# maybeLx/MVSFormerPlusPlus

Measured on AMD Instinct MI355X. Metric: ref-views/sec at 1152x1536 N=5 D=192 4-stage; achieved HBM GB/s vs peak, higher is better.
Workload: dtype fp16 operands/storage, fp32 accumulate (every stage; 1-2 fp16 MFMA terms)

## Files before the change

### mvsformerplusplus_amd/csrc/conv_bf16x3_kernels.hip

```cpp
#include <map>
#include <mutex>
#include <type_traits>
#include <utility>

#include "conv_cfg.h"
#include "split_format.h"

namespace mvs {

template <class Base>
struct F16Cfg : Base { static constexpr int ACT_F16 = 1; };
template <class Base>
struct F16x1Cfg : Base { static constexpr int ACT_F16 = 2; };
template <class Cfg, class = void> struct CfgFmt { static constexpr bool F16 = false, ONE = false; };
template <class Cfg> struct CfgFmt<Cfg, decltype((void)Cfg::ACT_F16)> { static constexpr bool F16 = true, ONE = Cfg::ACT_F16 == 2; };
typedef _Float16 f16x8 __attribute__((ext_vector_type(8)));
typedef _Float16 f16x4 __attribute__((ext_vector_type(4)));

__device__ __forceinline__ f16x4 f16_pack4(const float4& v, float& amax) {
    const float m = 65504.0f;
    sat::track(amax, v.x, v.y, v.z, v.w);
    return f16x4{(_Float16)__builtin_amdgcn_fmed3f(v.x, -m, m), (_Float16)__builtin_amdgcn_fmed3f(v.y, -m, m),
                 (_Float16)__builtin_amdgcn_fmed3f(v.z, -m, m), (_Float16)__builtin_amdgcn_fmed3f(v.w, -m, m)};
}
// ... 261 lines not shown
            __builtin_amdgcn_sched_barrier(0);
            if constexpr ((T & 1) == 0) bf_mfma_step<Cfg::MREP, Cfg::NREP, CfgFmt<Cfg>::F16, CfgFmt<Cfg>::ONE>(ah, al, bh0, bl0, acc);
            else bf_mfma_step<Cfg::MREP, Cfg::NREP, CfgFmt<Cfg>::F16, CfgFmt<Cfg>::ONE>(ah, al, bh1, bl1, acc);
            if constexpr (T % W::WC == W::WC - 1) {
                if (gc + 1 < nchunk_total) bf_wlds_store<Cfg>(ring, gc + 1, tid, piece);
                __syncthreads();
            }
            BfWldsSteps<Cfg, T + 1>::run(g, lane, tid, wp, ring, gc0, nchunk_total, mb0, ldsb, voxbase0, acc, piece, bh0, bl0, bh1, bl1);
        }
    }
};

template <class Cfg, bool SPLIT>
__global__ __launch_bounds__(256) void conv3d_mfma_bf16x3_kernel(const float* __restrict__ x, const void* wp, const float* __restrict__ bias,
                                                                 float* __restrict__ y, int D, int H, int W, int OD, int OH, int OW,
                                                                 int relu, int tiles_x, int tiles_y, int ntiles) {
    float sat_amax = 0.0f;
    constexpr int CIN = Cfg::CIN, COUT = Cfg::COUT, SD = Cfg::SD, SH = Cfg::SH, SW = Cfg::SW, TD = Cfg::TD, TH = Cfg::TH, CH = Cfg::CH;
    constexpr int IH = Cfg::IH, IW = Cfg::IW, MREP = Cfg::MREP, NREP = Cfg::NREP;
    constexpr int OPT = BfConv<Cfg>::OPT, NSTEP = BfConv<Cfg>::NSTEP, SB = BfConv<Cfg>::SB;
    HIP_DYNAMIC_SHARED(float4, lds4)
    char* ldsb = reinterpret_cast<char*>(lds4);
    const int tid = (int)threadIdx.x, lane = tid & 63, wave = tid >> 6;
    const int li = lane & 15, g = lane >> 4;
    int tile = (int)xcd_remap(blockIdx.x, (unsigned)ntiles);
    const int b = (int)blockIdx.y;
    const int tx = tile % tiles_x;
    tile /= tiles_x;
    const int ty = tile % tiles_y, tz = tile / tiles_y;
    const int oz0 = tz * TD, oy0 = ty * TH, ox0 = tx * 16;
    const int iz0 = oz0 * SD - Cfg::PD, iy0 = oy0 * SH - 1, ix0 = ox0 * SW - 1;

    f32x4 acc[MREP][NREP];
#pragma unroll
    for (int mb = 0; mb < MREP; ++mb)
#pragma unroll
        for (int nb = 0; nb < NREP; ++nb) acc[mb][nb] = (f32x4){0.0f, 0.0f, 0.0f, 0.0f};

    constexpr int MSPLIT = CfgSplit<Cfg>::MSPLIT, MREP_ALL = CfgSplit<Cfg>::MREP_ALL;
    const int mb0 = (wave % MSPLIT) * MREP, rowgrp = wave / MSPLIT;
    int voxbase[NREP];
#pragma unroll
    for (int nb = 0; nb < NREP; ++nb) {
        const int nbg = rowgrp * NREP + nb;
// ... 116 lines not shown
                else bf_conv_load_x<Cfg, T + 1>(g, ldsb, voxbase0, bh0, bl0);
            }
            __builtin_amdgcn_sched_barrier(0);
            const bf16x8* a_hi = BfConv<Cfg>::PERSIST_WLDS ? aw : wh[T];
            const bf16x8* a_lo = BfConv<Cfg>::PERSIST_WLDS ? aw : wl[T];
            if constexpr ((T & 1) == 0) bf_mfma_step<Cfg::MREP, Cfg::NREP, CfgFmt<Cfg>::F16, CfgFmt<Cfg>::ONE>(a_hi, a_lo, bh0, bl0, acc);
            else bf_mfma_step<Cfg::MREP, Cfg::NREP, CfgFmt<Cfg>::F16, CfgFmt<Cfg>::ONE>(a_hi, a_lo, bh1, bl1, acc);
            BfConvStepsWreg<Cfg, T + 1>::run(g, wh, wl, ldsb, voxbase0, acc, bh0, bl0, bh1, bl1, wlane);
        }
    }
};

template <class Cfg, bool SPLIT>
__global__ __launch_bounds__(256) void conv3d_mfma_bf16x3_persist_kernel(const float* __restrict__ x, const void* wp, const float* __restrict__ bias,
                                                                         float* __restrict__ y, float* __restrict__ logits, int D, int H, int W,
                                                                         int OD, int OH, int OW, int relu, int tiles_x, int tiles_y, int ntiles) {
    float sat_amax = 0.0f;
    constexpr int CIN = Cfg::CIN, COUT = Cfg::COUT, SD = Cfg::SD, SH = Cfg::SH, SW = Cfg::SW, TD = Cfg::TD, TH = Cfg::TH;
    constexpr int IH = Cfg::IH, IW = Cfg::IW, MREP = Cfg::MREP, NREP = Cfg::NREP;
    constexpr int OPT = BfConv<Cfg>::OPT, NSTEP = BfConv<Cfg>::NSTEP, SB = BfConv<Cfg>::SB;
    static_assert(Cfg::NPASS == 1, "the persistent form keeps one channel chunk's weights in registers");
    HIP_DYNAMIC_SHARED(float4, lds4)
    char* ldsb = reinterpret_cast<char*>(lds4);
    const int tid = (int)threadIdx.x, lane = tid & 63, wave = tid >> 6;
    const int li = lane & 15, g = lane >> 4;
    const int b = (int)blockIdx.y;
    const int nblk = (int)gridDim.x, per = (ntiles + nblk - 1) / nblk;
    const int t_begin = (int)xcd_remap(blockIdx.x, (unsigned)nblk) * per;
    const int t_end = t_begin + per < ntiles ? t_begin + per : ntiles;
    if (t_begin >= t_end) return;

    const bf16x8* wq = reinterpret_cast<const bf16x8*>(wp) + lane;
    bf16x8 wh[NSTEP][MREP], wl[NSTEP][MREP];
    constexpr bool WL = BfConv<Cfg>::PERSIST_WLDS;
    const char* wlane = ldsb + BfConv<Cfg>::WLDS_OFF + lane * 16;
    if constexpr (WL) {
        bf16x8* dst = reinterpret_cast<bf16x8*>(ldsb + BfConv<Cfg>::WLDS_OFF);
        for (int i = tid; i < NSTEP * MREP * 64; i += 256) dst[i] = reinterpret_cast<const bf16x8*>(wp)[(size_t)((i >> 6) * 2) * 64 + (i & 63)];
    } else {
#pragma unroll
        for (int t = 0; t < NSTEP; ++t)
#pragma unroll
            for (int mb = 0; mb < MREP; ++mb) {
                wh[t][mb] = wq[(size_t)((t * MREP + mb) * 2) * 64];
// ... 7 lines not shown
    int voxbase[NREP];
#pragma unroll
    for (int nb = 0; nb < NREP; ++nb) {
        const int nbg = wave * NREP + nb;
        const int oz = nbg / TH, oy = nbg % TH;
        voxbase[nb] = (((oz * SD) * IH + oy * SH) * IW + li * SW) * SB;
    }
    constexpr bool F16 = BfConv<Cfg>::F16;
    constexpr int EB = F16 ? 2 : 4, RUNB = BfConv<Cfg>::RUNB;
    const char* xb = reinterpret_cast<const char*>(x) + (size_t)b * D * H * W * CIN * EB;
    char* yb = y ? reinterpret_cast<char*>(y) + (size_t)b * OD * OH * OW * COUT * EB : nullptr;

    constexpr int NITEM = Cfg::NVOX * OPT, NIT = (NITEM + 255) / 256;
    float4 su[NIT], sv[NIT];
    auto issue = [&](int tile) {
        const int tx = tile % tiles_x;
        const int t1 = tile / tiles_x;
        const int ty = t1 % tiles_y, tz = t1 / tiles_y;
        const int iz0 = tz * TD * SD - Cfg::PD, iy0 = ty * TH * SH - 1, ix0 = tx * 16 * SW - 1;
        int zrel;
        const __amdgpu_buffer_rsrc_t xrs = bf_make_rsrc_z(xb, iz0, D, H, W, (unsigned)(CIN * EB), zrel);
        BfTileWalk<IW, IH, OPT, RUNB> wk(tid, zrel, iy0, ix0, H, W, CIN * EB, 0u);
#pragma unroll
        for (int it = 0; it < NIT; ++it) {
            if (it > 0) wk.advance();
            const bool ok = (it * 256 + 255 < NITEM || tid + it * 256 < NITEM) && wk.inside(iz0, iy0, ix0, D, H, W);
            const unsigned voff = ok ? wk.off : BF_OOB;
            su[it] = bf_buf_load16(xrs, voff, 0);
            if constexpr (!F16) sv[it] = bf_buf_load16(xrs, voff, 16);
        }
    };
    auto process = [&](int tile) {
#pragma unroll
        for (int it = 0; it < NIT; ++it) {
            const int e = tid + it * 256;
            if (e >= NITEM) break;
            const int vox = e / OPT, oc = e - vox * OPT;
            if constexpr (F16) *reinterpret_cast<float4*>(ldsb + vox * SB + oc * BfConv<Cfg>::PLANE) = su[it];
            else stage_to_lds<SPLIT>(ldsb + vox * SB + oc * BfConv<Cfg>::PLANE, su[it], sv[it]);
        }
        __syncthreads();
        if (tile + 1 < t_end) issue(tile + 1);

        f32x4 acc[MREP][NREP];
#pragma unroll
        for (int mb = 0; mb < MREP; ++mb)
#pragma unroll
            for (int nb = 0; nb < NREP; ++nb) acc[mb][nb] = (f32x4){0.0f, 0.0f, 0.0f, 0.0f};
        {
            bf16x8 bh0[NREP], bl0[NREP], bh1[NREP], bl1[NREP];
            bf_conv_load_x<Cfg, 0>(g, ldsb, voxbase[0], bh0, bl0);
            BfConvStepsWreg<Cfg, 0>::run(g, wh, wl, ldsb, voxbase[0], acc, bh0, bl0, bh1, bl1, wlane);
        }

        const int tx = tile % tiles_x;
        const int t1 = tile / tiles_x;
        const int ty = t1 % tiles_y, tz = t1 / tiles_y;
        const int oz0 = tz * TD, oy0 = ty * TH, ox0 = tx * 16;
#pragma unroll
        for (int nb = 0; nb < NREP; ++nb) {
            const int nbg = wave * NREP + nb;
            const int oz = oz0 + nbg / TH, oy = oy0 + nbg % TH, ox = ox0 + li;
            const bool inside = oz < OD && oy < OH && ox < OW;
            if (!inside && (!SPLIT || logits != nullptr)) continue;
            if (logits != nullptr) {
                if (g == 0) logits[(size_t)b * OD * OH * OW + ((size_t)oz * OH + oy) * OW + ox] = acc[0][nb][0] + bb[0].x;
                continue;
            }
            float* o = reinterpret_cast<float*>(yb + (((size_t)oz * OH + oy) * OW + ox) * COUT * EB);
#pragma unroll
            for (int mb = 0; mb < MREP; ++mb) {
                const int co = 16 * mb + 4 * g;
                if (!SPLIT && co >= COUT) continue;
                float4 v = make_float4(acc[mb][nb][0] + bb[mb].x, acc[mb][nb][1] + bb[mb].y, acc[mb][nb][2] + bb[mb].z, acc[mb][nb][3] + bb[mb].w);
                if (relu) { v.x = fmaxf(v.x, 0.0f); v.y = fmaxf(v.y, 0.0f); v.z = fmaxf(v.z, 0.0f); v.w = fmaxf(v.w, 0.0f); }
                if constexpr (F16) *reinterpret_cast<f16x4*>(reinterpret_cast<_Float16*>(o) + co) = f16_pack4(v, sat_amax);
                else if (SPLIT) split_store_quad(o + (co & ~7), g, v, inside && co < COUT);
                else *reinterpret_cast<float4*>(o + co) = v;
            }
        }
        __syncthreads();
    };
    issue(t_begin);
    for (int tile = t_begin; tile < t_end; ++tile) process(tile);
    if constexpr (F16) sat::commit(sat_amax);
}


template <class Cfg>
struct BfDeconv {
    static constexpr int OPT = Cfg::CIN / 8;
    static constexpr bool F16 = CfgFmt<Cfg>::F16;
    static constexpr int RUNB = F16 ? 16 : 32;
    static constexpr int SB = F16 ? 16 : 32;
    static constexpr int PLANE = F16 ? (Cfg::NVOX * 16 + 255) / 256 * 256 + bf_f16_plane_shift(1)
                                     : (Cfg::NVOX * 32 + 255) / 256 * 256 + 16;
    static constexpr size_t LDS_BYTES = (size_t)OPT * PLANE;
};

// ... 125 lines not shown
            bfdf_mfma_all<Cfg, U, P::F16 ? 1 : 2>(ah, al, bh[U & 1], bl[U & 1], acc);
            if constexpr (NEXT) {
                __builtin_amdgcn_sched_barrier(0);
                bfdf_load_w_all<Cfg, U + 1, 2, 1>(wrs, wvoff, ah, al);
            }
            BfDeconvFSteps<Cfg, U + 1>::run(wrs, wvoff, px, acc, ah, al, bh, bl);
        }
    }
};

template <class Cfg, bool SPLIT, bool FUSED = false>
__global__ __launch_bounds__(256) void deconv3d_mfma_bf16x3_kernel(const float* __restrict__ x, const void* wp, const float* __restrict__ bias,
                                                                   const float* __restrict__ skip, float* __restrict__ y,
                                                                   const float* __restrict__ prob_w, const float* __restrict__ prob_b,
                                                                   float* __restrict__ logits, int D, int H, int W, int tiles_x,
                                                                   int tiles_y, int ntiles, int relu) {
    float sat_amax = 0.0f;
    constexpr int CIN = Cfg::CIN, COUT = Cfg::COUT, SD = Cfg::SD, TDM = Cfg::TDM, THM = Cfg::THM;
    constexpr int LH = Cfg::LH, LW = Cfg::LW, MREP = Cfg::MREP, NREP = Cfg::NREP;
    constexpr int OPT = BfDeconv<Cfg>::OPT, SB = BfDeconv<Cfg>::SB;
    const float lo_clamp = relu ? 0.0f : -INFINITY;
    HIP_DYNAMIC_SHARED(float4, lds4)
    char* ldsb = reinterpret_cast<char*>(lds4);
    const int tid = (int)threadIdx.x, lane = tid & 63, wave = tid >> 6;
    const int li = lane & 15, g = lane >> 4;
    int tile = (int)xcd_remap(blockIdx.x, (unsigned)ntiles);
    const int b = (int)blockIdx.y;
    const int tx = tile % tiles_x;
    tile /= tiles_x;
    const int ty = tile % tiles_y, tz = tile / tiles_y;
    const int mz0 = tz * TDM, my0 = ty * THM, mx0 = tx * 16;
    const int OD = D * SD, OH = 2 * H, OW = 2 * W;

    constexpr bool F16 = BfDeconv<Cfg>::F16;
    constexpr int EB = F16 ? 2 : 4, RUNB = BfDeconv<Cfg>::RUNB;
    const char* xb = reinterpret_cast<const char*>(x) + (size_t)b * D * H * W * CIN * EB;
    {
        int zrel;
        const __amdgpu_buffer_rsrc_t xrs = bf_make_rsrc_z(xb, mz0 - Cfg::ZO, D, H, W, (unsigned)(CIN * EB), zrel);
        BfTileWalk<LW, LH, OPT, RUNB> wk(tid, zrel, my0, mx0, H, W, CIN * EB, 0u);
        int ldso = (tid / OPT) * SB + (tid % OPT) * BfDeconv<Cfg>::PLANE;
        for (int e = tid; e < Cfg::NVOX * OPT; e += 256) {
            const bool ok = wk.inside(mz0 - Cfg::ZO, my0, mx0, D, H, W);
            const unsigned voff = ok ? wk.off : BF_OOB;
            const float4 u = bf_buf_load16(xrs, voff, 0);
// ... 222 lines not shown
                else bfd_load_step<Cfg, IT, T + 1>(g, lane, ldsx, ldsw, voxbase0, a0[0], a0[1], bh0, bl0);
            }
            __builtin_amdgcn_sched_barrier(0);
            if constexpr ((T & 1) == 0) bf_mfma_step<1, Cfg::NREP, CfgFmt<Cfg>::F16, CfgFmt<Cfg>::ONE>(&a0[0], &a0[1], bh0, bl0, acc);
            else bf_mfma_step<1, Cfg::NREP, CfgFmt<Cfg>::F16, CfgFmt<Cfg>::ONE>(&a1[0], &a1[1], bh1, bl1, acc);
            BfDeconvSteps<Cfg, IT, T + 1>::run(g, lane, ldsx, ldsw, voxbase0, acc, a0, bh0, bl0, a1, bh1, bl1);
        }
    }
};

template <class Cfg, bool SPLIT>
__global__ __launch_bounds__(256) void deconv3d_mfma_bf16x3_persist_kernel(const float* __restrict__ x, const void* wp, const float* __restrict__ bias,
                                                                           const float* __restrict__ skip, float* __restrict__ y,
                                                                           const float* __restrict__ prob_w, const float* __restrict__ prob_b,
                                                                           float* __restrict__ logits, int D, int H, int W, int tiles_x, int tiles_y,
                                                                           int ntiles, int relu) {
    float sat_amax = 0.0f;
    using P = BfDeconvP<Cfg>;
    const float lo_clamp = relu ? 0.0f : -INFINITY;
    constexpr int CIN = Cfg::CIN, COUT = Cfg::COUT, SD = Cfg::SD, TDM = Cfg::TDM, THM = Cfg::THM;
    constexpr int LH = Cfg::LH, LW = Cfg::LW, NREP = Cfg::NREP, NIT = P::NIT, OPT = P::OPT, SB = P::SB;
    HIP_DYNAMIC_SHARED(float4, lds4)
    char* ldsx = reinterpret_cast<char*>(lds4);
    char* ldsw = ldsx + P::XBYTES;
    const int tid = (int)threadIdx.x, lane = tid & 63, wave = tid >> 6;
    const int li = lane & 15, g = lane >> 4;
    const int b = (int)blockIdx.y;
    const int nblk = (int)gridDim.x, per = (ntiles + nblk - 1) / nblk;
    const int t_begin = (int)xcd_remap(blockIdx.x, (unsigned)nblk) * per;
    const int t_end = t_begin + per < ntiles ? t_begin + per : ntiles;
    if (t_begin >= t_end) return;
    const int OD = D * SD, OH = 2 * H, OW = 2 * W;

    for (int e = tid; e < P::WBYTES / 16; e += 256) reinterpret_cast<float4*>(ldsw)[e] = reinterpret_cast<const float4*>(wp)[e];

    constexpr bool F16 = P::F16;
    constexpr int EB = F16 ? 2 : 4;
    const char* xb = reinterpret_cast<const char*>(x) + (size_t)b * D * H * W * CIN * EB;
    float* yb = y ? reinterpret_cast<float*>(reinterpret_cast<char*>(y) + (size_t)b * OD * OH * OW * COUT * EB) : nullptr;
    const float* sb = skip ? reinterpret_cast<const float*>(reinterpret_cast<const char*>(skip) + (size_t)b * OD * OH * OW * COUT * EB) : nullptr;
    const int co = 4 * (g & 1);
    const float4 bb = *reinterpret_cast<const float4*>(bias + co);
    const bool head = prob_w != nullptr;
    const float4 pw4 = head ? *reinterpret_cast<const float4*>(prob_w + co) : make_float4(0.0f, 0.0f, 0.0f, 0.0f);
    const float pb = head ? prob_b[0] : 0.0f;

    int voxbase[NREP];
#pragma unroll
    for (int nb = 0; nb < NREP; ++nb) {
        const int nbg = wave * NREP + nb;
        const int mz = nbg / THM, my = nbg % THM;
        voxbase[nb] = (((mz + Cfg::ZO) * LH + my) * LW + li) * SB;
    }

    constexpr int NITEM = Cfg::NVOX * OPT, NITX = (NITEM + 255) / 256;
    float4 su[NITX], sv[NITX];
    auto issue_x = [&](int tile) {
        const int tx = tile % tiles_x;
        const int t1 = tile / tiles_x;
        const int ty = t1 % tiles_y, tz = t1 / tiles_y;
        const int mz0 = tz * TDM, my0 = ty * THM, mx0 = tx * 16;
        int zrel;
        const __amdgpu_buffer_rsrc_t xrs = bf_make_rsrc_z(xb, mz0 - Cfg::ZO, D, H, W, (unsigned)(CIN * EB), zrel);
        BfTileWalk<LW, LH, OPT, P::RUNB> wk(tid, zrel, my0, mx0, H, W, CIN * EB, 0u);
#pragma unroll
        for (int it = 0; it < NITX; ++it) {
            if (it > 0) wk.advance();
            const bool ok = (it * 256 + 255 < NITEM || tid + it * 256 < NITEM) && wk.inside(mz0 - Cfg::ZO, my0, mx0, D, H, W);
            const unsigned voff = ok ? wk.off : BF_OOB;
            su[it] = bf_buf_load16(xrs, voff, 0);
            if constexpr (!F16) sv[it] = bf_buf_load16(xrs, voff, 16);
        }
    };
    float4 skp[NIT][NREP];
    auto issue_skip = [&](int tile) {
        const int tx = tile % tiles_x;
        const int t1 = tile / tiles_x;
        const int ty = t1 % tiles_y, tz = t1 / tiles_y;
        const int mz0 = tz * TDM, my0 = ty * THM, mx0 = tx * 16;
#pragma unroll
        for (int it = 0; it < NIT; ++it) {
            const int pd = (SD == 2) ? (it >> 1) : 0, ph = it & 1;
#pragma unroll
            for (int nb = 0; nb < NREP; ++nb) {
                const int nbg = wave * NREP + nb;
                const int mz = mz0 + nbg / THM, my = my0 + nbg % THM, mx = mx0 + li;
                const bool inside = mz < D && my < H && mx < W;
                const int oz = mz * SD + pd, oy = 2 * my + ph, ox = 2 * mx + (g >> 1);
                const size_t vbase = inside ? (((size_t)oz * OH + oy) * OW + ox) * COUT : 0;
                if constexpr (F16) {
                    const float2 raw = *reinterpret_cast<const float2*>(reinterpret_cast<const _Float16*>(sb) + vbase + co);
                    skp[it][nb] = inside ? make_float4(raw.x, raw.y, 0.0f, 0.0f) : make_float4(0.0f, 0.0f, 0.0f, 0.0f);
                    continue;
                }
                const float4 sk = SPLIT ? split_raw_quad(sb + vbase, co >> 2) : *reinterpret_cast<const float4*>(sb + vbase + co);
                skp[it][nb] = inside ? sk : make_float4(0.0f, 0.0f, 0.0f, 0.0f);
            }
        }
    };
    issue_x(t_begin);
    if (sb) issue_skip(t_begin);
    for (int tile = t_begin; tile < t_end; ++tile) {
#pragma unroll
        for (int it = 0; it < NITX; ++it) {
            const int e = tid + it * 256;
            if (e >= NITEM) break;
            const int vox = e / OPT, oc = e - vox * OPT;
            if constexpr (F16) *reinterpret_cast<float4*>(ldsx + vox * SB + oc * P::PLANE) = su[it];
            else stage_to_lds<SPLIT>(ldsx + vox * SB + oc * P::PLANE, su[it], sv[it]);
        }
        __syncthreads();
        if (tile + 1 < t_end) issue_x(tile + 1);

        const int tx = tile % tiles_x;
        const int t1 = tile / tiles_x;
        const int ty = t1 % tiles_y, tz = t1 / tiles_y;
        const int mz0 = tz * TDM, my0 = ty * THM, mx0 = tx * 16;
        float4 outv[NIT][NREP];
        auto run_class = [&](auto itc) {
            constexpr int IT = decltype(itc)::value;
            f32x4 acc[1][NREP];
#pragma unroll
            for (int nb = 0; nb < NREP; ++nb) acc[0][nb] = (f32x4){0.0f, 0.0f, 0.0f, 0.0f};
            bf16x8 a0[2], a1[2], bh0[NREP], bl0[NREP], bh1[NREP], bl1[NREP];
            bfd_load_step<Cfg, IT, 0>(g, lane, ldsx, ldsw, voxbase[0], a0[0], a0[1], bh0, bl0);
            BfDeconvSteps<Cfg, IT, 0>::run(g, lane, ldsx, ldsw, voxbase[0], acc, a0, bh0, bl0, a1, bh1, bl1);
#pragma unroll
            for (int nb = 0; nb < NREP; ++nb)
                outv[IT][nb] = make_float4(fmaxf(acc[0][nb][0] + bb.x, lo_clamp), fmaxf(acc[0][nb][1] + bb.y, lo_clamp), fmaxf(acc[0][nb][2] + bb.z, lo_clamp),
                                           fmaxf(acc[0][nb][3] + bb.w, lo_clamp));
        };
// ... 23 lines not shown
                    part += v.z * pw4.z;
                    part += v.w * pw4.w;
                    part += __shfl_xor(part, 16);
                    if ((g & 1) == 0 && inside)
                        logits[(size_t)b * OD * OH * OW + ((size_t)oz * OH + oy) * OW + ox] = part + pb;
                } else if (F16) {
                    if (inside) *reinterpret_cast<f16x4*>(reinterpret_cast<_Float16*>(yb) + (((size_t)oz * OH + oy) * OW + ox) * COUT + co) =
                        f16_pack4(v, sat_amax);
                } else if (SPLIT) {
                    split_store_quad(yb + (((size_t)oz * OH + oy) * OW + ox) * COUT, g, v, inside);
                } else if (inside) {
                    *reinterpret_cast<float4*>(yb + (((size_t)oz * OH + oy) * OW + ox) * COUT + co) = v;
                }
            }
        }
        if (sb && tile + 1 < t_end) issue_skip(tile + 1);
        __syncthreads();
    }
    if constexpr (F16) sat::commit(sat_amax);
}

static int resident_blocks(const void* func, size_t lds, int threads = 256) {
    static std::mutex mu;
    static std::map<std::pair<const void*, int>, int> cache;
    int dev = 0;
    if (hipGetDevice(&dev) != hipSuccess) return -1;
    std::lock_guard<std::mutex> lock(mu);
    auto it = cache.find(std::make_pair(func, dev));
    if (it != cache.end()) return it->second;
    int per_cu = 0;
    hipDeviceProp_t prop;
    if (lds > 48 * 1024) hipFuncSetAttribute(func, hipFuncAttributeMaxDynamicSharedMemorySize, (int)lds);
    if (hipGetDeviceProperties(&prop, dev) != hipSuccess || hipOccupancyMaxActiveBlocksPerMultiprocessor(&per_cu, func, threads, lds) != hipSuccess || per_cu < 1)
        return -1;
    return cache[std::make_pair(func, dev)] = per_cu * prop.multiProcessorCount;
}

constexpr int BF_MSPLIT_MIN_MREP = 4;
template <class Cfg>
struct BfSplitOf {
    static constexpr bool SPLIT = Cfg::MREP >= BF_MSPLIT_MIN_MREP && Cfg::NREP <= 2 && Cfg::TH % (Cfg::NREP * 2) == 0;
    typedef typename std::conditional<SPLIT, SplitCfg<Cfg, 2>, Cfg>::type type;
};

template <class Cfg, bool SPLIT>
static int launch_conv_bf(const float* x, const void* wp, const float* bias, float* y, int B, int D, int H, int W, int relu, hipStream_t st,
                          float* logits) {
    const int OD = (D + 2 * Cfg::PD - Cfg::KD) / Cfg::SD + 1, OH = (H - 1) / Cfg::SH + 1, OW = (W - 1) / Cfg::SW + 1;
    const int tx = (int)ceil_div(OW, 16), ty = (int)ceil_div(OH, Cfg::TH), tz = (int)ceil_div(OD, Cfg::TD);
    const int ntiles = tx * ty * tz;
    constexpr size_t LDS = BfConv<Cfg>::PERSIST ? BfConv<Cfg>::PERSIST_LDS_BYTES : BfConv<Cfg>::LDS_BYTES;
    if constexpr (BfConv<Cfg>::PERSIST) {
        const int resident = resident_blocks(reinterpret_cast<const void*>(&conv3d_mfma_bf16x3_persist_kernel<Cfg, SPLIT>), LDS);
        if (resident < 1) { set_error("conv3d(bf16x3): occupancy query failed"); return MVS_ERR_LAUNCH; }
        const int nblk = ntiles < resident ? ntiles : resident;
        hipLaunchKernelGGL((conv3d_mfma_bf16x3_persist_kernel<Cfg, SPLIT>), dim3(nblk, B), dim3(256), LDS, st, x, wp, bias, y, logits, D, H, W, OD, OH, OW, relu, tx,
                           ty, ntiles);
        return check_launch("conv3d_mfma_bf16x3_persist_kernel");
    }
    if (logits != nullptr) { set_error("conv3d(bf16x3): the planar single-channel output needs a persistent (Cin = 8) kernel"); return MVS_ERR_UNSUPPORTED; }
    constexpr size_t TLDS = BfWlds<Cfg>::ENABLED ? BfWlds<Cfg>::LDS_BYTES : LDS;
    if (TLDS > 48 * 1024)
        hipFuncSetAttribute(reinterpret_cast<const void*>(&conv3d_mfma_bf16x3_kernel<Cfg, SPLIT>), hipFuncAttributeMaxDynamicSharedMemorySize, (int)TLDS);
    hipLaunchKernelGGL((conv3d_mfma_bf16x3_kernel<Cfg, SPLIT>), dim3(ntiles, B), dim3(256), TLDS, st, x, wp, bias, y, D, H, W, OD, OH, OW, relu, tx, ty, ntiles);
    return check_launch("conv3d_mfma_bf16x3_kernel");
}

template <class Cfg>
struct BfDeconvSplitOf {
    static constexpr bool SPLIT = Cfg::MREP == 2 && Cfg::THM % (Cfg::NREP * 2) == 0;
    typedef typename std::conditional<SPLIT, SplitCfg<Cfg, 2>, Cfg>::type type;
};

template <class Cfg, bool SPLIT>
static int launch_deconv_bf(const float* x, const void* wp, const float* bias, const float* skip, float* y, const float* prob_w,
                            const float* prob_b, float* logits, int B, int D, int H, int W, hipStream_t st, int relu) {
    const int tx = (int)ceil_div(W, 16), ty = (int)ceil_div(H, Cfg::THM), tz = (int)ceil_div(D, Cfg::TDM);
    const int ntiles = tx * ty * tz;
    if constexpr (Cfg::CIN == 16 && Cfg::COUT == 8) {
        constexpr size_t LDS = BfDeconvP<Cfg>::LDS_BYTES;
        const int resident = resident_blocks(reinterpret_cast<const void*>(&deconv3d_mfma_bf16x3_persist_kernel<Cfg, SPLIT>), LDS);
        if (resident < 1) { set_error("deconv3d(bf16x3): occupancy query failed"); return MVS_ERR_LAUNCH; }
        const int nblk = ntiles < resident ? ntiles : resident;
        hipLaunchKernelGGL((deconv3d_mfma_bf16x3_persist_kernel<Cfg, SPLIT>), dim3(nblk, B), dim3(256), LDS, st, x, wp, bias, skip, y, prob_w, prob_b, logits, D, H,
                           W, tx, ty, ntiles, relu);
        return check_launch("deconv3d_mfma_bf16x3_persist_kernel");
    }
    constexpr size_t DLDS = BfDeconv<Cfg>::LDS_BYTES;
    if constexpr (BfDeconvF<Cfg>::ENABLED) {
        const char* sw = getenv("MVS_DECONV_CLASS_FUSED");
        const bool fused = (sw == nullptr || sw[0] == '\0') ? BfDeconvF<Cfg>::DEFAULT : sw[0] != '0';
        if (fused) {
            if (DLDS > 48 * 1024)
                hipFuncSetAttribute(reinterpret_cast<const void*>(&deconv3d_mfma_bf16x3_kernel<Cfg, SPLIT, true>), hipFuncAttributeMaxDynamicSharedMemorySize, (int)DLDS);
            hipLaunchKernelGGL((deconv3d_mfma_bf16x3_kernel<Cfg, SPLIT, true>), dim3(ntiles, B), dim3(256), DLDS, st, x, wp, bias, skip, y, prob_w, prob_b,
                               logits, D, H, W, tx, ty, ntiles, relu);
            return check_launch("deconv3d_mfma_bf16x3_kernel");
        }
    }
    if (DLDS > 48 * 1024)
        hipFuncSetAttribute(reinterpret_cast<const void*>(&deconv3d_mfma_bf16x3_kernel<Cfg, SPLIT>), hipFuncAttributeMaxDynamicSharedMemorySize, (int)DLDS);
    hipLaunchKernelGGL((deconv3d_mfma_bf16x3_kernel<Cfg, SPLIT>), dim3(ntiles, B), dim3(256), DLDS, st, x, wp, bias, skip, y, prob_w, prob_b,
                       logits, D, H, W, tx, ty, ntiles, relu);
    return check_launch("deconv3d_mfma_bf16x3_kernel");
}

static bool bf_input_fits(const char* who, int Cin, int D, int H, int W, int split) {
    const long long bytes = 12LL * H * W * Cin * (split >= 2 ? 2 : 4);
    if (bytes < (1LL << 31)) return true;
    set_error("%s: twelve z-planes of the input are %lld bytes; the MFMA convolutions address a tile's planes with 32-bit offsets (< 2 GB)", who, bytes);
    return false;
}

int conv3d_dispatch_bf16x3(const float* x, const void* wp, const float* bias, float* y, int B, int Cin, int Cout, int D, int H, int W,
                           int kd, int sd, int sh, int sw, int relu, hipStream_t st, float* logits, int split) {
    if (!bf_input_fits("conv3d(mfma)", Cin, D, H, W, split)) return MVS_ERR_UNSUPPORTED;
#define MVS_X(CI, CO, KD, SD, SH, SW, TD, TH, CH)                                                     \
    if (Cin == CI && Cout == CO && kd == KD && sd == SD && sh == SH && sw == SW) {                    \
// ... 34 lines not shown
```

### mvsformerplusplus_amd/csrc/head_kernels.hip

```cpp
#include "mvs_common.h"

namespace mvs {

template <int DC>
__device__ __forceinline__ void head_from_logits(const float* l, const float* lg, const float* hp, size_t HW, int D, float tmp, int mode, int conf_n,
                                                 float* pv, float& depth, float& conf) {
#define HL(d) (DC > 0 ? l[(DC > 0 ? (d) : 0)] : lg[(size_t)(d) * HW])
    float m = -INFINITY;
#pragma unroll
    for (int d = 0; d < D; ++d) m = fmaxf(m, HL(d));
    float den = 0.0f;
#pragma unroll
    for (int d = 0; d < D; ++d) den += expf(HL(d) - m);

    depth = 0.0f;
    conf = 0.0f;
    if (mode == MVS_HEAD_CE_EVAL) {
        float m2 = -INFINITY;
#pragma unroll
        for (int d = 0; d < D; ++d) m2 = fmaxf(m2, HL(d) * tmp);
        float den2 = 0.0f;
#pragma unroll
        for (int d = 0; d < D; ++d) den2 += expf(HL(d) * tmp - m2);
#pragma unroll
// ... 224 lines not shown
            const float dmax = dep + (float)D / 2.0f * itv;
            lo[k] = dmin;
            span[k] = (dmax - dmin) / (float)(D - 1);
        }
    }
    for (int d = 0; d < D; ++d) {
        float c[4];
#pragma unroll
        for (int k = 0; k < 4; ++k)
            c[k] = linear ? lo[k] + (float)d * span[k] : lo[k] + span[k] * ((float)d / (float)(D - 1));
        const float v = ly0 * (lx0 * c[0] + lx1 * c[1]) + ly1 * (lx0 * c[2] + lx1 * c[3]);
        hyp[((size_t)b * D + d) * HW + p] = linear ? v : 1.0f / v;
    }
}

constexpr int HS_SH = 8, HS_SW = 32, HS_RH = HS_SH + 2, HS_RW = HS_SW + 2, HS_NREG = HS_RH * HS_RW;

template <int DC>
__global__ __launch_bounds__(256) void prob_regress_sched_kernel(const float* __restrict__ logits, const float* __restrict__ hyp, float tmp, int mode,
                                                                 int conf_n, float* __restrict__ depth_out, float* __restrict__ conf_out,
                                                                 float* __restrict__ prob_vol, int D_, int H, int W, float ratio,
                                                                 float* __restrict__ next_hyp, int Dn, int tiles_x) {
    __shared__ float s_lo[HS_NREG], s_span[HS_NREG];
    const int D = DC > 0 ? DC : D_;
    const size_t HW = (size_t)H * W;
    const int b = (int)blockIdx.y;
    const int ty = (int)blockIdx.x / tiles_x, tx = (int)blockIdx.x - ty * tiles_x;
    const int y0 = ty * HS_SH, x0 = tx * HS_SW;
    for (int task = (int)threadIdx.x; task < HS_NREG; task += 256) {
        const int ry = task / HS_RW, rx = task - ry * HS_RW;
        const int y = y0 - 1 + ry, x = x0 - 1 + rx;
        if (y < 0 || y >= H || x < 0 || x >= W) continue;
        const bool owner = ry >= 1 && ry <= HS_SH && rx >= 1 && rx <= HS_SW;
        const size_t p = (size_t)y * W + x;
        const float* lg = logits + (size_t)b * D * HW + p;
        const float* hp = hyp + (size_t)b * D * HW + p;
        float l[DC > 0 ? DC : 1];
        if (DC > 0) {
#pragma unroll
            for (int d = 0; d < (DC > 0 ? DC : 1); ++d) l[d] = lg[(size_t)d * HW];
        }
        float depth, conf;
// ... 134 lines not shown
        if (!cp.p[i] || cp.shift[i] < 0 || cp.shift[i] > 16 || ((H >> cp.shift[i]) << cp.shift[i]) != H || ((W >> cp.shift[i]) << cp.shift[i]) != W) {
            set_error("mvs_softmax_regress_confavg_fwd: earlier stage %d must be a 2^shift-times smaller map of this %dx%d stage", i, H, W);
            return MVS_ERR_ARG;
        }
    return launch_head<0>(logits, nullptr, nullptr, hyp, tmp, mode, conf_n, depth, conf, prob_volume, const_cast<float*>(logits), B, D, H, W, (hipStream_t)stream, cp, conf_avg);
}

extern "C" int mvs_softmax_regress_schedule_fwd(const float* logits, const float* hyp, float tmp, int mode, int conf_n, float* depth, float* conf,
                                               float* prob_volume, float ratio, float* next_hyp, int next_D, int B, int D, int H, int W, void* stream) {
    int rc = check_head("mvs_softmax_regress_schedule_fwd", logits, hyp, depth, conf, mode, B, D, H, W);
    if (rc != MVS_OK) return rc;
    if (!next_hyp || next_D < 2 || D < 3 || H < 2 || W < 2) { set_error("mvs_softmax_regress_schedule_fwd: bad arguments (needs D >= 3 hypotheses, module.py:708, and next_D >= 2)"); return MVS_ERR_ARG; }
    const int tiles_x = (int)ceil_div(W, HS_SW), tiles_y = (int)ceil_div(H, HS_SH);
    const dim3 grid(tiles_x * tiles_y, B), block(256);
    hipStream_t st = (hipStream_t)stream;
#define MVS_HS_CASE(DC)                                                                                                                   \
    case DC:                                                                                                                              \
        hipLaunchKernelGGL((prob_regress_sched_kernel<DC>), grid, block, 0, st, logits, hyp, tmp, mode, conf_n, depth, conf, prob_volume, D, H, W, ratio, \
                           next_hyp, next_D, tiles_x);                                                                                    \
        break;
    switch (D) {
        MVS_HS_CASE(4)
        MVS_HS_CASE(8)
        MVS_HS_CASE(16)
        MVS_HS_CASE(32)
        MVS_HS_CASE(48)
        default:
            hipLaunchKernelGGL((prob_regress_sched_kernel<0>), grid, block, 0, st, logits, hyp, tmp, mode, conf_n, depth, conf, prob_volume, D, H, W, ratio,
                               next_hyp, next_D, tiles_x);
    }
#undef MVS_HS_CASE
    return check_launch("prob_regress_sched_kernel");
}

extern "C" int mvs_depth_regression_fwd(const float* p, const float* depth_values, float* out, int B, int D, int H, int W, void* stream) {
    if (!p || !depth_values || !out || B < 1 || D < 1 || H < 1 || W < 1) { set_error("mvs_depth_regression_fwd: bad arguments"); return MVS_ERR_ARG; }
    hipLaunchKernelGGL(depth_regression_kernel, dim3(ceil_div((long long)H * W, 256), B), dim3(256), 0, (hipStream_t)stream, p, depth_values, out, D, H * W);
    return check_launch("depth_regression_kernel");
}

extern "C" int mvs_conf_regression_fwd(const float* p, int n, float* out, int B, int D, int H, int W, void* stream) {
    if (!p || !out || n < 1 || B < 1 || D < 1 || H < 1 || W < 1) { set_error("mvs_conf_regression_fwd: bad arguments"); return MVS_ERR_ARG; }
    hipLaunchKernelGGL(conf_regression_kernel, dim3(ceil_div((long long)H * W, 256), B), dim3(256), 0, (hipStream_t)stream, p, n, out, D, H * W);
    return check_launch("conf_regression_kernel");
// ... 58 lines not shown
```

### mvsformerplusplus_amd/csrc/mvs_common.h

```cpp
#pragma once
#include <hip/hip_runtime.h>

#include <stdint.h>

#include "../../include/mvs_hip.h"

#ifndef MVS_GLOBAL_LOAD_LDS16
#define MVS_GLOBAL_LOAD_LDS16(gsrc, ldst) \
    __builtin_amdgcn_global_load_lds((const __attribute__((address_space(1))) void*)(gsrc), (__attribute__((address_space(3))) void*)(ldst), 16, 0, 0)
#define MVS_WAIT_VMEM() asm volatile("s_waitcnt vmcnt(0)" ::: "memory")
#endif

#ifndef MVS_FMA_MIX_LO
namespace mvs {
__device__ __forceinline__ float fma_mix_lo(unsigned h2, float w, float acc) {
    float r;
    asm("v_fma_mix_f32 %0, %1, %2, %3 op_sel_hi:[1,0,0]" : "=v"(r) : "v"(h2), "v"(w), "v"(acc));
    return r;
}
__device__ __forceinline__ float fma_mix_hi(unsigned h2, float w, float acc) {
    float r;
    asm("v_fma_mix_f32 %0, %1, %2, %3 op_sel:[1,0,0] op_sel_hi:[1,0,0]" : "=v"(r) : "v"(h2), "v"(w), "v"(acc));
    return r;
}
// ... 28 lines not shown
}
#define MVS_DEFINE_SAT_READER(fn)                                                        \
    unsigned int fn(int reset) {                                                         \
        unsigned int v = 0;                                                              \
        if (hipMemcpyFromSymbol(&v, HIP_SYMBOL(mvs::sat::counter), sizeof(v)) != hipSuccess) return 0; \
        if (reset && v) { const unsigned int z = 0; hipMemcpyToSymbol(HIP_SYMBOL(mvs::sat::counter), &z, sizeof(z)); } \
        return v;                                                                        \
    }

constexpr int kWave = 64;
constexpr int kBlock = 256;
constexpr int kMaxSrcViews = 16;

void set_error(const char* fmt, ...);
int check_launch(const char* what);

template <int DT> struct FeatT;
template <> struct FeatT<MVS_DTYPE_F32> { typedef float type; };
template <> struct FeatT<MVS_DTYPE_BF16> { typedef uint16_t type; };
template <> struct FeatT<MVS_DTYPE_F16> { typedef _Float16 type; };

__device__ __forceinline__ float to_f32(float v) { return v; }
__device__ __forceinline__ float to_f32(_Float16 v) { return (float)v; }
__device__ __forceinline__ float to_f32(uint16_t bf16_bits) {
    union { uint32_t u; float f; } c;
    c.u = ((uint32_t)bf16_bits) << 16;
    return c.f;
}

template <typename T> __device__ __forceinline__ T from_f32(float v);
// ... 132 lines not shown
    int xb = x0, yb = y0;
    float wa = wx0, wb = wx1, wt = wy0, wd = wy1;
    if ((unsigned)x0 > (unsigned)(W - 2) || (unsigned)y0 > (unsigned)(H - 2)) {
        xb = x0 < 0 ? 0 : (x0 > W - 2 ? W - 2 : x0);
        yb = y0 < 0 ? 0 : (y0 > H - 2 ? H - 2 : y0);
        wa = x0 < 0 ? wx1 : (x0 > W - 2 ? 0.0f : wx0);
        wb = x0 < 0 ? 0.0f : (x0 > W - 2 ? wx0 : wx1);
        wt = y0 < 0 ? wy1 : (y0 > H - 2 ? 0.0f : wy0);
        wd = y0 < 0 ? 0.0f : (y0 > H - 2 ? wy0 : wy1);
    }
    tp.pk = ((unsigned)yb << 16) | (unsigned)xb;
    tp.w00 = wa * wt; tp.w01 = wb * wt; tp.w10 = wa * wd; tp.w11 = wb * wd;
    return tp;
}

__device__ __forceinline__ unsigned xcd_remap(unsigned b, unsigned n) {
    const unsigned q = n >> 3, r = n & 7u, xcd = b & 7u, idx = b >> 3;
    const unsigned base = (xcd < r) ? xcd * (q + 1) : r * (q + 1) + (xcd - r) * q;
    return base + idx;
}

static inline unsigned ceil_div(long long a, long long b) { return (unsigned)((a + b - 1) / b); }

__device__ __forceinline__ float init_range_value(float first, float last, int inverse, int d, int D) {
    if (inverse) {
        const float inv_min = 1.0f / first, inv_max = 1.0f / last;
        const float itv = (float)d / (float)(D - 1);
        return 1.0f / (inv_max + (inv_min - inv_max) * itv);
    }
    const float interval = (last - first) / (float)(D - 1);
    return first + (float)d * interval;
}

}
```

Baseline: 700.8.

## Reorder conv/deconv/head tiles into row bands for cross-XCD cache locality

Adds a banded tile ordering: tiles are decoded so that a few rows of y, spanning all x and z tiles, are handled together. The band height is sized so each band's working set fits in about 1 MiB of cache. Persistent kernels now take tiles with a stride inside an XCD group instead of a contiguous run. The goal is more L2/MALL reuse of halo rows between neighbouring tiles on the same XCD, which should cut HBM traffic. It is on by default for selected configs, can be switched off with an environment variable, and adds index arithmetic per tile plus a different load balance.

```diff
diff --git a/mvsformerplusplus_amd/csrc/conv_bf16x3_kernels.hip b/mvsformerplusplus_amd/csrc/conv_bf16x3_kernels.hip
--- a/mvsformerplusplus_amd/csrc/conv_bf16x3_kernels.hip
+++ b/mvsformerplusplus_amd/csrc/conv_bf16x3_kernels.hip
@@ -299,7 +299,7 @@
 template <class Cfg, bool SPLIT>
 __global__ __launch_bounds__(256) void conv3d_mfma_bf16x3_kernel(const float* __restrict__ x, const void* wp, const float* __restrict__ bias,
                                                                  float* __restrict__ y, int D, int H, int W, int OD, int OH, int OW,
-                                                                 int relu, int tiles_x, int tiles_y, int ntiles) {
+                                                                 int relu, int tiles_x, int tiles_y, int tiles_z, int band) {
     float sat_amax = 0.0f;
     constexpr int CIN = Cfg::CIN, COUT = Cfg::COUT, SD = Cfg::SD, SH = Cfg::SH, SW = Cfg::SW, TD = Cfg::TD, TH = Cfg::TH, CH = Cfg::CH;
     constexpr int IH = Cfg::IH, IW = Cfg::IW, MREP = Cfg::MREP, NREP = Cfg::NREP;
@@ -308,11 +308,9 @@
     char* ldsb = reinterpret_cast<char*>(lds4);
     const int tid = (int)threadIdx.x, lane = tid & 63, wave = tid >> 6;
     const int li = lane & 15, g = lane >> 4;
-    int tile = (int)xcd_remap(blockIdx.x, (unsigned)ntiles);
     const int b = (int)blockIdx.y;
-    const int tx = tile % tiles_x;
-    tile /= tiles_x;
-    const int ty = tile % tiles_y, tz = tile / tiles_y;
+    int tx, ty, tz;
+    tile_decode((int)xcd_remap(blockIdx.x, gridDim.x), tiles_x, tiles_y, tiles_z, band, tx, ty, tz);
     const int oz0 = tz * TD, oy0 = ty * TH, ox0 = tx * 16;
     const int iz0 = oz0 * SD - Cfg::PD, iy0 = oy0 * SH - 1, ix0 = ox0 * SW - 1;
 
@@ -459,7 +457,8 @@
 template <class Cfg, bool SPLIT>
 __global__ __launch_bounds__(256) void conv3d_mfma_bf16x3_persist_kernel(const float* __restrict__ x, const void* wp, const float* __restrict__ bias,
                                                                          float* __restrict__ y, float* __restrict__ logits, int D, int H, int W,
-                                                                         int OD, int OH, int OW, int relu, int tiles_x, int tiles_y, int ntiles) {
+                                                                         int OD, int OH, int OW, int relu, int tiles_x, int tiles_y, int tiles_z,
+                                                                         int band) {
     float sat_amax = 0.0f;
     constexpr int CIN = Cfg::CIN, COUT = Cfg::COUT, SD = Cfg::SD, SH = Cfg::SH, SW = Cfg::SW, TD = Cfg::TD, TH = Cfg::TH;
     constexpr int IH = Cfg::IH, IW = Cfg::IW, MREP = Cfg::MREP, NREP = Cfg::NREP;
@@ -470,9 +469,8 @@
     const int tid = (int)threadIdx.x, lane = tid & 63, wave = tid >> 6;
     const int li = lane & 15, g = lane >> 4;
     const int b = (int)blockIdx.y;
-    const int nblk = (int)gridDim.x, per = (ntiles + nblk - 1) / nblk;
-    const int t_begin = (int)xcd_remap(blockIdx.x, (unsigned)nblk) * per;
-    const int t_end = t_begin + per < ntiles ? t_begin + per : ntiles;
+    const TileRun trun = tile_run((int)blockIdx.x, (int)gridDim.x, tiles_x * tiles_y * tiles_z, band);
+    const int t_begin = trun.first, t_end = trun.end, t_step = trun.stride;
     if (t_begin >= t_end) return;
 
     const bf16x8* wq = reinterpret_cast<const bf16x8*>(wp) + lane;
@@ -510,9 +508,8 @@
     constexpr int NITEM = Cfg::NVOX * OPT, NIT = (NITEM + 255) / 256;
     float4 su[NIT], sv[NIT];
     auto issue = [&](int tile) {
-        const int tx = tile % tiles_x;
-        const int t1 = tile / tiles_x;
-        const int ty = t1 % tiles_y, tz = t1 / tiles_y;
+        int tx, ty, tz;
+        tile_decode(tile, tiles_x, tiles_y, tiles_z, band, tx, ty, tz);
         const int iz0 = tz * TD * SD - Cfg::PD, iy0 = ty * TH * SH - 1, ix0 = tx * 16 * SW - 1;
         int zrel;
         const __amdgpu_buffer_rsrc_t xrs = bf_make_rsrc_z(xb, iz0, D, H, W, (unsigned)(CIN * EB), zrel);
@@ -536,7 +533,7 @@
             else stage_to_lds<SPLIT>(ldsb + vox * SB + oc * BfConv<Cfg>::PLANE, su[it], sv[it]);
         }
         __syncthreads();
-        if (tile + 1 < t_end) issue(tile + 1);
+        if (tile + t_step < t_end) issue(tile + t_step);
 
         f32x4 acc[MREP][NREP];
 #pragma unroll
@@ -549,9 +546,8 @@
             BfConvStepsWreg<Cfg, 0>::run(g, wh, wl, ldsb, voxbase[0], acc, bh0, bl0, bh1, bl1, wlane);
         }
 
-        const int tx = tile % tiles_x;
-        const int t1 = tile / tiles_x;
-        const int ty = t1 % tiles_y, tz = t1 / tiles_y;
+        int tx, ty, tz;
+        tile_decode(tile, tiles_x, tiles_y, tiles_z, band, tx, ty, tz);
         const int oz0 = tz * TD, oy0 = ty * TH, ox0 = tx * 16;
 #pragma unroll
         for (int nb = 0; nb < NREP; ++nb) {
@@ -578,7 +574,7 @@
         __syncthreads();
     };
     issue(t_begin);
-    for (int tile = t_begin; tile < t_end; ++tile) process(tile);
+    for (int tile = t_begin; tile < t_end; tile += t_step) process(tile);
     if constexpr (F16) sat::commit(sat_amax);
 }
 
@@ -734,7 +730,7 @@
                                                                    const float* __restrict__ skip, float* __restrict__ y,
                                                                    const float* __restrict__ prob_w, const float* __restrict__ prob_b,
                                                                    float* __restrict__ logits, int D, int H, int W, int tiles_x,
-                                                                   int tiles_y, int ntiles, int relu) {
+                                                                   int tiles_y, int tiles_z, int band, int relu) {
     float sat_amax = 0.0f;
     constexpr int CIN = Cfg::CIN, COUT = Cfg::COUT, SD = Cfg::SD, TDM = Cfg::TDM, THM = Cfg::THM;
     constexpr int LH = Cfg::LH, LW = Cfg::LW, MREP = Cfg::MREP, NREP = Cfg::NREP;
@@ -744,11 +740,9 @@
     char* ldsb = reinterpret_cast<char*>(lds4);
     const int tid = (int)threadIdx.x, lane = tid & 63, wave = tid >> 6;
     const int li = lane & 15, g = lane >> 4;
-    int tile = (int)xcd_remap(blockIdx.x, (unsigned)ntiles);
     const int b = (int)blockIdx.y;
-    const int tx = tile % tiles_x;
-    tile /= tiles_x;
-    const int ty = tile % tiles_y, tz = tile / tiles_y;
+    int tx, ty, tz;
+    tile_decode((int)xcd_remap(blockIdx.x, gridDim.x), tiles_x, tiles_y, tiles_z, band, tx, ty, tz);
     const int mz0 = tz * TDM, my0 = ty * THM, mx0 = tx * 16;
     const int OD = D * SD, OH = 2 * H, OW = 2 * W;
 
@@ -1001,7 +995,7 @@
                                                                            const float* __restrict__ skip, float* __restrict__ y,
                                                                            const float* __restrict__ prob_w, const float* __restrict__ prob_b,
                                                                            float* __restrict__ logits, int D, int H, int W, int tiles_x, int tiles_y,
-                                                                           int ntiles, int relu) {
+                                                                           int tiles_z, int band, int relu) {
     float sat_amax = 0.0f;
     using P = BfDeconvP<Cfg>;
     const float lo_clamp = relu ? 0.0f : -INFINITY;
@@ -1013,9 +1007,8 @@
     const int tid = (int)threadIdx.x, lane = tid & 63, wave = tid >> 6;
     const int li = lane & 15, g = lane >> 4;
     const int b = (int)blockIdx.y;
-    const int nblk = (int)gridDim.x, per = (ntiles + nblk - 1) / nblk;
-    const int t_begin = (int)xcd_remap(blockIdx.x, (unsigned)nblk) * per;
-    const int t_end = t_begin + per < ntiles ? t_begin + per : ntiles;
+    const TileRun trun = tile_run((int)blockIdx.x, (int)gridDim.x, tiles_x * tiles_y * tiles_z, band);
+    const int t_begin = trun.first, t_end = trun.end, t_step = trun.stride;
     if (t_begin >= t_end) return;
     const int OD = D * SD, OH = 2 * H, OW = 2 * W;
 
@@ -1043,9 +1036,8 @@
     constexpr int NITEM = Cfg::NVOX * OPT, NITX = (NITEM + 255) / 256;
     float4 su[NITX], sv[NITX];
     auto issue_x = [&](int tile) {
-        const int tx = tile % tiles_x;
-        const int t1 = tile / tiles_x;
-        const int ty = t1 % tiles_y, tz = t1 / tiles_y;
+        int tx, ty, tz;
+        tile_decode(tile, tiles_x, tiles_y, tiles_z, band, tx, ty, tz);
         const int mz0 = tz * TDM, my0 = ty * THM, mx0 = tx * 16;
         int zrel;
         const __amdgpu_buffer_rsrc_t xrs = bf_make_rsrc_z(xb, mz0 - Cfg::ZO, D, H, W, (unsigned)(CIN * EB), zrel);
@@ -1061,9 +1053,8 @@
     };
     float4 skp[NIT][NREP];
     auto issue_skip = [&](int tile) {
-        const int tx = tile % tiles_x;
-        const int t1 = tile / tiles_x;
-        const int ty = t1 % tiles_y, tz = t1 / tiles_y;
+        int tx, ty, tz;
+        tile_decode(tile, tiles_x, tiles_y, tiles_z, band, tx, ty, tz);
         const int mz0 = tz * TDM, my0 = ty * THM, mx0 = tx * 16;
 #pragma unroll
         for (int it = 0; it < NIT; ++it) {
@@ -1087,7 +1078,7 @@
     };
     issue_x(t_begin);
     if (sb) issue_skip(t_begin);
-    for (int tile = t_begin; tile < t_end; ++tile) {
+    for (int tile = t_begin; tile < t_end; tile += t_step) {
 #pragma unroll
         for (int it = 0; it < NITX; ++it) {
             const int e = tid + it * 256;
@@ -1097,11 +1088,10 @@
             else stage_to_lds<SPLIT>(ldsx + vox * SB + oc * P::PLANE, su[it], sv[it]);
         }
         __syncthreads();
-        if (tile + 1 < t_end) issue_x(tile + 1);
-
-        const int tx = tile % tiles_x;
-        const int t1 = tile / tiles_x;
-        const int ty = t1 % tiles_y, tz = t1 / tiles_y;
+        if (tile + t_step < t_end) issue_x(tile + t_step);
+
+        int tx, ty, tz;
+        tile_decode(tile, tiles_x, tiles_y, tiles_z, band, tx, ty, tz);
         const int mz0 = tz * TDM, my0 = ty * THM, mx0 = tx * 16;
         float4 outv[NIT][NREP];
         auto run_class = [&](auto itc) {
@@ -1155,7 +1145,7 @@
                 }
             }
         }
-        if (sb && tile + 1 < t_end) issue_skip(tile + 1);
+        if (sb && tile + t_step < t_end) issue_skip(tile + t_step);
         __syncthreads();
     }
     if constexpr (F16) sat::commit(sat_amax);
@@ -1177,6 +1167,26 @@
     return cache[std::make_pair(func, dev)] = per_cu * prop.multiProcessorCount;
 }
 
+int tile_order_band(long long row_bytes, bool dflt_new) {
+    const char* sw = getenv("MVS_TILE_ORDER");
+    if (sw == nullptr || sw[0] == '\0') return dflt_new ? tile_band_rows(row_bytes) : 0;
+    if (sw[0] == '0') return 0;
+    if (sw[1] == ':') {
+        const int n = atoi(sw + 2);
+        if (n >= 1) return n;
+    }
+    return tile_band_rows(row_bytes);
+}
+
+template <class Cfg>
+struct BfTileOrder {
+    static constexpr bool NEW_CONV = !BfConv<Cfg>::PERSIST && Cfg::TD == 2 && Cfg::SD == 1;
+};
+template <class Cfg>
+struct BfDeconvTileOrder {
+    static constexpr bool NEW = !(Cfg::CIN == 16 && Cfg::COUT == 8) && Cfg::TDM == 2 && Cfg::SD == 1;
+};
+
 constexpr int BF_MSPLIT_MIN_MREP = 4;
 template <class Cfg>
 struct BfSplitOf {
@@ -1190,20 +1200,22 @@
     const int OD = (D + 2 * Cfg::PD - Cfg::KD) / Cfg::SD + 1, OH = (H - 1) / Cfg::SH + 1, OW = (W - 1) / Cfg::SW + 1;
     const int tx = (int)ceil_div(OW, 16), ty = (int)ceil_div(OH, Cfg::TH), tz = (int)ceil_div(OD, Cfg::TD);
     const int ntiles = tx * ty * tz;
+    constexpr int EBT = BfConv<Cfg>::F16 ? 2 : 4;
+    const int band = tile_order_band((long long)tx * tz * (Cfg::NVOX * Cfg::CIN + Cfg::TD * Cfg::TH * 16 * Cfg::COUT) * EBT, BfTileOrder<Cfg>::NEW_CONV);
     constexpr size_t LDS = BfConv<Cfg>::PERSIST ? BfConv<Cfg>::PERSIST_LDS_BYTES : BfConv<Cfg>::LDS_BYTES;
     if constexpr (BfConv<Cfg>::PERSIST) {
         const int resident = resident_blocks(reinterpret_cast<const void*>(&conv3d_mfma_bf16x3_persist_kernel<Cfg, SPLIT>), LDS);
         if (resident < 1) { set_error("conv3d(bf16x3): occupancy query failed"); return MVS_ERR_LAUNCH; }
         const int nblk = ntiles < resident ? ntiles : resident;
         hipLaunchKernelGGL((conv3d_mfma_bf16x3_persist_kernel<Cfg, SPLIT>), dim3(nblk, B), dim3(256), LDS, st, x, wp, bias, y, logits, D, H, W, OD, OH, OW, relu, tx,
-                           ty, ntiles);
+                           ty, tz, band);
         return check_launch("conv3d_mfma_bf16x3_persist_kernel");
     }
     if (logits != nullptr) { set_error("conv3d(bf16x3): the planar single-channel output needs a persistent (Cin = 8) kernel"); return MVS_ERR_UNSUPPORTED; }
     constexpr size_t TLDS = BfWlds<Cfg>::ENABLED ? BfWlds<Cfg>::LDS_BYTES : LDS;
     if (TLDS > 48 * 1024)
         hipFuncSetAttribute(reinterpret_cast<const void*>(&conv3d_mfma_bf16x3_kernel<Cfg, SPLIT>), hipFuncAttributeMaxDynamicSharedMemorySize, (int)TLDS);
-    hipLaunchKernelGGL((conv3d_mfma_bf16x3_kernel<Cfg, SPLIT>), dim3(ntiles, B), dim3(256), TLDS, st, x, wp, bias, y, D, H, W, OD, OH, OW, relu, tx, ty, ntiles);
+    hipLaunchKernelGGL((conv3d_mfma_bf16x3_kernel<Cfg, SPLIT>), dim3(ntiles, B), dim3(256), TLDS, st, x, wp, bias, y, D, H, W, OD, OH, OW, relu, tx, ty, tz, band);
     return check_launch("conv3d_mfma_bf16x3_kernel");
 }
 
@@ -1218,13 +1230,16 @@
                             const float* prob_b, float* logits, int B, int D, int H, int W, hipStream_t st, int relu) {
     const int tx = (int)ceil_div(W, 16), ty = (int)ceil_div(H, Cfg::THM), tz = (int)ceil_div(D, Cfg::TDM);
     const int ntiles = tx * ty * tz;
+    constexpr int EBT = BfDeconv<Cfg>::F16 ? 2 : 4;
+    const int band = tile_order_band((long long)tx * tz * (Cfg::NVOX * Cfg::CIN + (skip ? 2 : 1) * Cfg::TDM * Cfg::SD * Cfg::THM * 64 * Cfg::COUT) * EBT,
+                                     BfDeconvTileOrder<Cfg>::NEW);
     if constexpr (Cfg::CIN == 16 && Cfg::COUT == 8) {
         constexpr size_t LDS = BfDeconvP<Cfg>::LDS_BYTES;
         const int resident = resident_blocks(reinterpret_cast<const void*>(&deconv3d_mfma_bf16x3_persist_kernel<Cfg, SPLIT>), LDS);
         if (resident < 1) { set_error("deconv3d(bf16x3): occupancy query failed"); return MVS_ERR_LAUNCH; }
         const int nblk = ntiles < resident ? ntiles : resident;
         hipLaunchKernelGGL((deconv3d_mfma_bf16x3_persist_kernel<Cfg, SPLIT>), dim3(nblk, B), dim3(256), LDS, st, x, wp, bias, skip, y, prob_w, prob_b, logits, D, H,
-                           W, tx, ty, ntiles, relu);
+                           W, tx, ty, tz, band, relu);
         return check_launch("deconv3d_mfma_bf16x3_persist_kernel");
     }
     constexpr size_t DLDS = BfDeconv<Cfg>::LDS_BYTES;
@@ -1235,14 +1250,14 @@
             if (DLDS > 48 * 1024)
                 hipFuncSetAttribute(reinterpret_cast<const void*>(&deconv3d_mfma_bf16x3_kernel<Cfg, SPLIT, true>), hipFuncAttributeMaxDynamicSharedMemorySize, (int)DLDS);
             hipLaunchKernelGGL((deconv3d_mfma_bf16x3_kernel<Cfg, SPLIT, true>), dim3(ntiles, B), dim3(256), DLDS, st, x, wp, bias, skip, y, prob_w, prob_b,
-                               logits, D, H, W, tx, ty, ntiles, relu);
+                               logits, D, H, W, tx, ty, tz, band, relu);
             return check_launch("deconv3d_mfma_bf16x3_kernel");
         }
     }
     if (DLDS > 48 * 1024)
         hipFuncSetAttribute(reinterpret_cast<const void*>(&deconv3d_mfma_bf16x3_kernel<Cfg, SPLIT>), hipFuncAttributeMaxDynamicSharedMemorySize, (int)DLDS);
     hipLaunchKernelGGL((deconv3d_mfma_bf16x3_kernel<Cfg, SPLIT>), dim3(ntiles, B), dim3(256), DLDS, st, x, wp, bias, skip, y, prob_w, prob_b,
-                       logits, D, H, W, tx, ty, ntiles, relu);
+                       logits, D, H, W, tx, ty, tz, band, relu);
     return check_launch("deconv3d_mfma_bf16x3_kernel");
 }
 
diff --git a/mvsformerplusplus_amd/csrc/head_kernels.hip b/mvsformerplusplus_amd/csrc/head_kernels.hip
--- a/mvsformerplusplus_amd/csrc/head_kernels.hip
+++ b/mvsformerplusplus_amd/csrc/head_kernels.hip
@@ -262,18 +262,20 @@
     }
 }
 
+constexpr bool HS_TILE_ORDER_NEW = true;
 constexpr int HS_SH = 8, HS_SW = 32, HS_RH = HS_SH + 2, HS_RW = HS_SW + 2, HS_NREG = HS_RH * HS_RW;
 
 template <int DC>
 __global__ __launch_bounds__(256) void prob_regress_sched_kernel(const float* __restrict__ logits, const float* __restrict__ hyp, float tmp, int mode,
                                                                  int conf_n, float* __restrict__ depth_out, float* __restrict__ conf_out,
                                                                  float* __restrict__ prob_vol, int D_, int H, int W, float ratio,
-                                                                 float* __restrict__ next_hyp, int Dn, int tiles_x) {
+                                                                 float* __restrict__ next_hyp, int Dn, int tiles_x, int tiles_y, int band) {
     __shared__ float s_lo[HS_NREG], s_span[HS_NREG];
     const int D = DC > 0 ? DC : D_;
     const size_t HW = (size_t)H * W;
     const int b = (int)blockIdx.y;
-    const int ty = (int)blockIdx.x / tiles_x, tx = (int)blockIdx.x - ty * tiles_x;
+    int tx, ty, tz;
+    tile_decode(band > 0 ? (int)xcd_remap(blockIdx.x, gridDim.x) : (int)blockIdx.x, tiles_x, tiles_y, 1, band, tx, ty, tz);
     const int y0 = ty * HS_SH, x0 = tx * HS_SW;
     for (int task = (int)threadIdx.x; task < HS_NREG; task += 256) {
         const int ry = task / HS_RW, rx = task - ry * HS_RW;
@@ -438,10 +440,12 @@
     const int tiles_x = (int)ceil_div(W, HS_SW), tiles_y = (int)ceil_div(H, HS_SH);
     const dim3 grid(tiles_x * tiles_y, B), block(256);
     hipStream_t st = (hipStream_t)stream;
+    const int band = tile_order_band((long long)tiles_x * 4 * ((2LL * HS_NREG + (prob_volume ? HS_SH * HS_SW : 0)) * D + 4LL * HS_SH * HS_SW * next_D),
+                                     HS_TILE_ORDER_NEW);
 #define MVS_HS_CASE(DC)                                                                                                                   \
     case DC:                                                                                                                              \
         hipLaunchKernelGGL((prob_regress_sched_kernel<DC>), grid, block, 0, st, logits, hyp, tmp, mode, conf_n, depth, conf, prob_volume, D, H, W, ratio, \
-                           next_hyp, next_D, tiles_x);                                                                                    \
+                           next_hyp, next_D, tiles_x, tiles_y, band);                                                                                    \
         break;
     switch (D) {
         MVS_HS_CASE(4)
@@ -451,7 +455,7 @@
         MVS_HS_CASE(48)
         default:
             hipLaunchKernelGGL((prob_regress_sched_kernel<0>), grid, block, 0, st, logits, hyp, tmp, mode, conf_n, depth, conf, prob_volume, D, H, W, ratio,
-                               next_hyp, next_D, tiles_x);
+                               next_hyp, next_D, tiles_x, tiles_y, band);
     }
 #undef MVS_HS_CASE
     return check_launch("prob_regress_sched_kernel");
diff --git a/mvsformerplusplus_amd/csrc/mvs_common.h b/mvsformerplusplus_amd/csrc/mvs_common.h
--- a/mvsformerplusplus_amd/csrc/mvs_common.h
+++ b/mvsformerplusplus_amd/csrc/mvs_common.h
@@ -4,6 +4,7 @@
 #include <stdint.h>
 
 #include "../../include/mvs_hip.h"
+#include "tile_order.h"
 
 #ifndef MVS_GLOBAL_LOAD_LDS16
 #define MVS_GLOBAL_LOAD_LDS16(gsrc, ldst) \
@@ -66,6 +67,7 @@
 
 void set_error(const char* fmt, ...);
 int check_launch(const char* what);
+int tile_order_band(long long row_bytes, bool dflt_new);
 
 template <int DT> struct FeatT;
 template <> struct FeatT<MVS_DTYPE_F32> { typedef float type; };
@@ -228,11 +230,6 @@
     return tp;
 }
 
-__device__ __forceinline__ unsigned xcd_remap(unsigned b, unsigned n) {
-    const unsigned q = n >> 3, r = n & 7u, xcd = b & 7u, idx = b >> 3;
-    const unsigned base = (xcd < r) ? xcd * (q + 1) : r * (q + 1) + (xcd - r) * q;
-    return base + idx;
-}
 
 static inline unsigned ceil_div(long long a, long long b) { return (unsigned)((a + b - 1) / b); }
 
diff --git a/mvsformerplusplus_amd/csrc/tile_order.h b/mvsformerplusplus_amd/csrc/tile_order.h
--- /dev/null
+++ b/mvsformerplusplus_amd/csrc/tile_order.h
@@ -0,0 +1,65 @@
+#pragma once
+
+#if defined(__HIPCC__)
+#define MVS_TILE_HD __host__ __device__ __forceinline__
+#else
+#define MVS_TILE_HD inline
+#endif
+
+namespace mvs {
+
+MVS_TILE_HD unsigned xcd_remap(unsigned b, unsigned n) {
+    const unsigned q = n >> 3, r = n & 7u, xcd = b & 7u, idx = b >> 3;
+    const unsigned base = (xcd < r) ? xcd * (q + 1) : r * (q + 1) + (xcd - r) * q;
+    return base + idx;
+}
+
+MVS_TILE_HD void tile_decode(int t, int tiles_x, int tiles_y, int tiles_z, int band, int& tx, int& ty, int& tz) {
+    if (band <= 0) {
+        tx = t % tiles_x;
+        t /= tiles_x;
+        ty = t % tiles_y;
+        tz = t / tiles_y;
+        return;
+    }
+    const int per_band = band * tiles_x * tiles_z;
+    const int bi = t / per_band;
+    int r = t - bi * per_band;
+    const int y0 = bi * band;
+    const int bh = tiles_y - y0 < band ? tiles_y - y0 : band;
+    tz = r % tiles_z;
+    r /= tiles_z;
+    ty = y0 + r % bh;
+    tx = r / bh;
+}
+
+struct TileRun {
+    int first, end, stride;
+};
+
+MVS_TILE_HD TileRun tile_run(int b, int nblk, int ntiles, int band) {
+    TileRun run;
+    if (band <= 0) {
+        const int per = (ntiles + nblk - 1) / nblk;
+        run.first = (int)xcd_remap((unsigned)b, (unsigned)nblk) * per;
+        run.end = run.first + per < ntiles ? run.first + per : ntiles;
+        run.stride = 1;
+        return run;
+    }
+    const int G = nblk < 8 ? nblk : 8;
+    const int grp = b % G, p = b / G;
+    const int n = (nblk - grp + G - 1) / G;
+    const int q = ntiles / G, r = ntiles % G;
+    const int base = grp < r ? grp * (q + 1) : r * (q + 1) + (grp - r) * q;
+    run.first = base + p;
+    run.end = base + q + (grp < r ? 1 : 0);
+    run.stride = n;
+    return run;
+}
+
+MVS_TILE_HD int tile_band_rows(long long row_bytes) {
+    const long long n = (1LL << 20) / (row_bytes > 0 ? row_bytes : 1);
+    return n < 1 ? 1 : n > 8 ? 8 : (int)n;
+}
+
+}
```

Result: no change. 702.0, median of 3 (+0.2%).
